# JohnsonLabJanelia/laserCalib

Hardware: NVIDIA B200
Metric: LM_iters_per_sec (higher is better)
Workload: dtype f64

## Files before the change

### include/lcba.h

```cpp
#ifndef LCBA_H
#define LCBA_H

#include <stddef.h>
#include <stdint.h>

#ifdef __cplusplus
extern "C" {
#endif

#define LCBA_VERSION 100
#define LCBA_CAM_PARAMS 11
#define LCBA_MAX_CAMERAS 64
#define LCBA_MAX_TRACE 512

enum {
  LCBA_OK = 0,
  LCBA_E_ARG = -1,
  LCBA_E_CUDA = -2,
  LCBA_E_STATE = -3,
  LCBA_E_UNSUPPORTED = -4,
  LCBA_E_NONFINITE = -5,
  LCBA_E_NCCL = -6
};

// ... 33 lines not shown

typedef struct lcba_result {
  double cost;
  double optimality;
  double initial_cost;
  int64_t nfev;
  int64_t njev;
  int64_t iterations;
  int32_t status;
  int32_t n_trace;
  double solve_ms;
  int64_t gpu_launches;
  double reserved[6];
} lcba_result;

typedef struct lcba_kernel_stat {
  char name[32];
  int64_t launches;
  double total_ms;
} lcba_kernel_stat;

int lcba_version(void);
int lcba_create(lcba_t** out, int device);
void lcba_destroy(lcba_t* h);
const char* lcba_last_error(const lcba_t* h);
void lcba_default_options(lcba_options* o);

int lcba_set_problem(lcba_t* h, int32_t C, int64_t P, int64_t N, const double* cams,
                     const double* pts, const double* obs_uv, const int64_t* cam_idx,
                     const int64_t* pt_idx, const double* weights_or_null);
int lcba_set_problem_shard(lcba_t* h, int32_t C, int64_t P, int64_t N, const double* cams,
                           const double* pts, const double* obs_uv, const int64_t* cam_idx,
                           const int64_t* pt_idx, const double* weights_or_null, int64_t pt_offset);
int lcba_set_params(lcba_t* h, const double* cams, const double* pts);
int lcba_get_params(lcba_t* h, double* cams_out, double* pts_out);

int lcba_rotate(lcba_t* h, int64_t M, const double* pts, const double* rot_vecs, double* out);
int lcba_project(lcba_t* h, int64_t M, const double* pts, const double* cams_rows,
                 double* out_uv);

int lcba_unproject(lcba_t* h, int64_t M, const double* uv, const double* Z, int64_t nZ,
                   const double* camera_matrix, const double* dist5, const double* rc_ext,
                   const double* tc_ext, double* out_xyz);

#define LCBA_SQ_CAMONLY 0
#define LCBA_SQ_TRANSFORM 1
int lcba_sq_normal(lcba_t* h, int32_t mode, const double* theta, double* cost_out, double* g_out,
                   double* H_out);

int lcba_residuals(lcba_t* h, const double* x_or_null, double* r_out, double* cost_out);

int lcba_jacobian_blocks(lcba_t* h, const double* x_or_null, double* Jc, double* Jp);

int lcba_sparsity_indices(lcba_t* h, int32_t C, int64_t P, int64_t N, const int64_t* cam_idx,
                          const int64_t* pt_idx, int32_t* indices_out);

int lcba_solve(lcba_t* h, const lcba_options* opt, lcba_result* res);
int lcba_get_trace(lcba_t* h, lcba_trace_row* rows, int32_t max_rows);
typedef void (*lcba_iteration_cb)(const lcba_trace_row* row, void* user);
int lcba_set_iteration_callback(lcba_t* h, lcba_iteration_cb cb, void* user);
int lcba_get_grad(lcba_t* h, double* g_out );
int lcba_get_profile(lcba_t* h, lcba_kernel_stat* stats, int32_t max_stats, int32_t* n_out);

int lcba_linearize(lcba_t* h, double lam, double* S_out, double* rhs_out, double* grad_out,
                   double* scale_inv_out, double* cost_out);

int lcba_time_device(lcba_t* h, int32_t what, int32_t reps, double* ms_out);

int lcba_nccl_unique_id(void* id_out128);
int lcba_comm_init(lcba_t* h, int32_t rank, int32_t nranks, const void* id128);

int lcba_debug_tr2d(double B00, double B01, double B11, double g0, double g1, double Delta,
                    double* p_out2, int* newton_out);

int lcba_debug_schur_stats(lcba_t* h, long long* out, int max_ctas, int* nkinds, int* nslices);

int lcba_debug_mma_plan(int32_t C, int32_t sm_count, int32_t* units_out, int32_t max_kinds,
                        int32_t* nslices_out, int32_t* ok_out);

int lcba_debug_i8_plan(int32_t C, int64_t P, int32_t sm_count, int32_t* tiles_out, int32_t max_tiles,
                       int32_t* work_out, int32_t max_work, int32_t* nwork_out, int32_t* nrg_out,
                       int64_t* nkb_out);

int lcba_debug_peer_reduce(lcba_t* h, int enable);

int lcba_host_is_nondecreasing_i64(const int64_t* v, int64_t n, int32_t threads);

#ifdef __cplusplus
}
#endif
#endif
```

### lasercalib_b200/_cabi.py

```python
from __future__ import annotations

import ctypes as C
import os

import numpy as np

_PKG = os.path.dirname(os.path.abspath(__file__))
LIB_PATH = os.path.join(_PKG, "liblcba.so")

LCBA_MAX_TRACE = 512
E_NAMES = {-1: "LCBA_E_ARG", -2: "LCBA_E_CUDA", -3: "LCBA_E_STATE", -4: "LCBA_E_UNSUPPORTED",
           -5: "LCBA_E_NONFINITE", -6: "LCBA_E_NCCL"}

SYMBOLS = ["lcba_version", "lcba_create", "lcba_destroy", "lcba_last_error", "lcba_default_options",
           "lcba_set_problem", "lcba_set_problem_shard", "lcba_set_params", "lcba_get_params", "lcba_rotate", "lcba_project",
           "lcba_unproject", "lcba_residuals", "lcba_jacobian_blocks", "lcba_sparsity_indices", "lcba_solve",
           "lcba_get_trace", "lcba_get_grad", "lcba_get_profile", "lcba_linearize",
           "lcba_time_device", "lcba_nccl_unique_id", "lcba_comm_init", "lcba_debug_tr2d",
           "lcba_sq_normal", "lcba_debug_schur_stats", "lcba_debug_mma_plan",
           "lcba_set_iteration_callback", "lcba_debug_i8_plan", "lcba_host_is_nondecreasing_i64", "lcba_debug_peer_reduce"]


class Options(C.Structure):
    _fields_ = [("ftol", C.c_double), ("xtol", C.c_double), ("gtol", C.c_double),
                ("max_nfev", C.c_int64), ("verbose", C.c_int32), ("profile", C.c_int32),
                ("max_iterations", C.c_int32), ("fix_cameras", C.c_int32), ("shared_intrinsics", C.c_int32), ("reserved", C.c_int32 * 3)]


class TraceRow(C.Structure):
    _fields_ = [("iteration", C.c_int64), ("nfev", C.c_int64), ("cost", C.c_double),
                ("cost_reduction", C.c_double), ("step_norm", C.c_double),
                ("optimality", C.c_double), ("delta", C.c_double), ("reg_term", C.c_double)]


class Result(C.Structure):
    _fields_ = [("cost", C.c_double), ("optimality", C.c_double), ("initial_cost", C.c_double),
                ("nfev", C.c_int64), ("njev", C.c_int64), ("iterations", C.c_int64),
                ("status", C.c_int32), ("n_trace", C.c_int32), ("solve_ms", C.c_double),
                ("gpu_launches", C.c_int64), ("reserved", C.c_double * 6)]


class KernelStat(C.Structure):
    _fields_ = [("name", C.c_char * 32), ("launches", C.c_int64), ("total_ms", C.c_double)]


ITERATION_CB = C.CFUNCTYPE(None, C.POINTER(TraceRow), C.c_void_p)


def _row_dict(r):
    return dict(iteration=r.iteration, nfev=r.nfev, cost=r.cost, cost_reduction=r.cost_reduction,
                step_norm=r.step_norm, optimality=r.optimality, delta=r.delta, reg_term=r.reg_term)


class LcbaError(RuntimeError):
    def __init__(self, code, msg):
        super().__init__("%s (%d): %s" % (E_NAMES.get(code, "LCBA_E_?"), code, msg))
        self.code = code


_lib = None


def load():
    global _lib
    if _lib is not None:
        return _lib
    if not os.path.exists(LIB_PATH):
        raise ImportError(
            "lasercalib_b200: %s is missing — build it with `python -m lasercalib_b200.build` "
            "(there is no CPU fallback)" % LIB_PATH)
    lib = C.CDLL(LIB_PATH, mode=C.RTLD_GLOBAL)
    vp, i32, i64, dbl = C.c_void_p, C.c_int32, C.c_int64, C.c_double
    pd = C.POINTER(C.c_double)
    lib.lcba_version.restype = C.c_int
    lib.lcba_create.argtypes = [C.POINTER(vp), C.c_int]
    lib.lcba_destroy.argtypes = [vp]
    lib.lcba_destroy.restype = None
    lib.lcba_last_error.argtypes = [vp]
    lib.lcba_last_error.restype = C.c_char_p
    lib.lcba_default_options.argtypes = [C.POINTER(Options)]
    lib.lcba_default_options.restype = None
    lib.lcba_set_problem.argtypes = [vp, i32, i64, i64, vp, vp, vp, vp, vp, vp]
    lib.lcba_set_problem_shard.argtypes = [vp, i32, i64, i64, vp, vp, vp, vp, vp, vp, i64]
    lib.lcba_set_params.argtypes = [vp, vp, vp]
    lib.lcba_get_params.argtypes = [vp, vp, vp]
    lib.lcba_rotate.argtypes = [vp, i64, vp, vp, vp]
    lib.lcba_project.argtypes = [vp, i64, vp, vp, vp]
    lib.lcba_unproject.argtypes = [vp, i64, vp, vp, i64, vp, vp, vp, vp, vp]
    lib.lcba_residuals.argtypes = [vp, vp, vp, pd]
    lib.lcba_jacobian_blocks.argtypes = [vp, vp, vp, vp]
    lib.lcba_sparsity_indices.argtypes = [vp, i32, i64, i64, vp, vp, vp]
    lib.lcba_solve.argtypes = [vp, C.POINTER(Options), C.POINTER(Result)]
    lib.lcba_get_trace.argtypes = [vp, C.POINTER(TraceRow), i32]
    lib.lcba_set_iteration_callback.argtypes = [vp, ITERATION_CB, vp]
    lib.lcba_get_grad.argtypes = [vp, vp]
    lib.lcba_get_profile.argtypes = [vp, C.POINTER(KernelStat), i32, C.POINTER(i32)]
    lib.lcba_linearize.argtypes = [vp, dbl, vp, vp, vp, vp, pd]
    lib.lcba_time_device.argtypes = [vp, i32, i32, pd]
    lib.lcba_nccl_unique_id.argtypes = [vp]
    lib.lcba_comm_init.argtypes = [vp, i32, i32, vp]
    lib.lcba_sq_normal.argtypes = [vp, i32, vp, pd, vp, vp]
    lib.lcba_debug_mma_plan.argtypes = [i32, i32, vp, i32, C.POINTER(i32), C.POINTER(i32)]
    lib.lcba_debug_schur_stats.argtypes = [vp, vp, C.c_int, C.POINTER(C.c_int), C.POINTER(C.c_int)]
    lib.lcba_debug_i8_plan.argtypes = [i32, i64, i32, vp, i32, vp, i32, C.POINTER(i32), C.POINTER(i32), C.POINTER(i64)]
    lib.lcba_host_is_nondecreasing_i64.argtypes = [vp, i64, i32]
    lib.lcba_debug_peer_reduce.argtypes = [vp, i32]
    lib.lcba_debug_tr2d.argtypes = [dbl, dbl, dbl, dbl, dbl, dbl, pd, C.POINTER(C.c_int)]
    _lib = lib
    return lib


def _ptr(a):
    return None if a is None else a.ctypes.data_as(C.c_void_p)


def _f64(a, shape=None):
    a = np.ascontiguousarray(a, dtype=np.float64)
    if shape is not None:
        a = a.reshape(shape)
    return a


def _i64(a):
    return np.ascontiguousarray(a, dtype=np.int64)


class Engine:

    def __init__(self, device=-1):
        self.lib = load()
        h = C.c_void_p()
        rc = self.lib.lcba_create(C.byref(h), int(device))
        if rc != 0:
            raise LcbaError(rc, self.lib.lcba_last_error(None).decode())
        self.h = h
        self.C = self.P = self.N = 0
        self.generation = 0

    def close(self):
        if getattr(self, "h", None):
            self.lib.lcba_destroy(self.h)
            self.h = None

    def __del__(self):
        try:
            self.close()
        except Exception:
            pass

    def _check(self, rc):
        if rc != 0:
            raise LcbaError(rc, self.lib.lcba_last_error(self.h).decode())

    def set_problem(self, cams, pts, points_2d, camera_ind, point_ind, weights=None, pt_offset=0):
        cams, pts = _f64(cams), _f64(pts)
        p2 = _f64(points_2d)
        ci, pi = _i64(camera_ind).ravel(), _i64(point_ind).ravel()
        w = None if weights is None else _f64(weights).ravel()
        if cams.ndim != 2 or cams.shape[1] != 11:
            raise ValueError("cameraArray must have shape (n_cameras, 11)")
        if pts.ndim != 2 or pts.shape[1] != 3:
            raise ValueError("points3D must have shape (n_points, 3)")
        N = ci.size
        if pi.size != N or p2.shape != (N, 2) or (w is not None and w.size != N):
            raise ValueError("observation arrays must share their first dimension")
        self._check(self.lib.lcba_set_problem_shard(self.h, cams.shape[0], pts.shape[0], N,
                                                    _ptr(cams), _ptr(pts), _ptr(p2), _ptr(ci),
                                                    _ptr(pi), _ptr(w), int(pt_offset)))
        self.C, self.P, self.N = cams.shape[0], pts.shape[0], N
        self.generation += 1

    def set_params(self, cams, pts):
        self.generation += 1
        cams, pts = _f64(cams, (self.C, 11)), _f64(pts, (self.P, 3))
        self._check(self.lib.lcba_set_params(self.h, _ptr(cams), _ptr(pts)))

    def get_params(self, x_out=None):
        if x_out is None:
            cams = np.empty((self.C, 11))
            pts = np.empty((self.P, 3))
        else:
            cams = x_out[: 11 * self.C].reshape(self.C, 11)
            pts = x_out[11 * self.C:].reshape(self.P, 3)
        self._check(self.lib.lcba_get_params(self.h, _ptr(cams), _ptr(pts)))
        return cams, pts

    def rotate(self, points, rot_vecs):
# ... 144 lines not shown
```

### lasercalib_b200/csrc/lcba.cu

```cuda
#include <dlfcn.h>
#include <math.h>
#include <stdio.h>
#include <string.h>
#include <algorithm>
#include <map>
#include <string>
#include <thread>
#include <vector>

#include <nvtx3/nvToolsExt.h>

#include "common.cuh"
#include "control.cuh"
#include "dense.cuh"
#include "eval.cuh"
#include "ingest.cuh"
#include "linearize.cuh"
#include "dense_passes.cuh"
#include "schur.cuh"
#include "schur_mma.cuh"
#include "schur_i8.cuh"
#include "peer_reduce.cuh"
#include "variants.cuh"

// ... 802 lines not shown
  NvtxRange nvtx_("lcba:linearize");
  const int C = h->C, w = h->cur;
  LCBA_TRY(build_tables(h, w));
  if (h->use_dense) {
    const size_t smem = dense_lin_smem_doubles(C) * 8;
    KL(h, "linearize", k_linearize_dense<<<h->dp_grid_lin, DP_THREADS, smem, h->stream>>>(
          h->d_tab[w], h->d_pts[w], h->d_uv, h->d_w, h->d_obs_start, h->d_mask, h->P, C, h->dp_pb,
          h->d_Vg, h->d_dpart, h->d_part));
    KL(h, "reduce", k_reduce_cols<<<nblk(C * DP_CAM_VALS, RC_COLS), RC_COLS * RC_ROWS, 0, h->stream>>>(
          h->d_dpart, h->dp_grid_lin, C * DP_CAM_VALS, h->d_dred));
    KL(h, "reduce", k_dense_cam_unpack<<<nblk(C * DP_CAM_VALS, 128), 128, 0, h->stream>>>(
          h->d_dred, C, h->d_camsum, h->d_U));
    KL(h, "reduce", k_reduce_scalars<<<1, 256, 0, h->stream>>>(h->d_part, h->dp_grid_lin, 1,
                                                               h->d_camsum + C * CAMSUM, 1));
  } else {
  const size_t smem = linearize_smem_doubles(C) * 8;
  KL(h, "linearize", k_linearize<<<h->lin_grid, LIN_THREADS, smem, h->stream>>>(
        h->d_tab[w], h->d_pts[w], h->d_uv, h->d_cam, h->d_pt, h->d_w, h->d_obs_start, h->d_bins,
        h->nbins, C, h->d_Vg, h->d_campart, h->d_part));
  KL(h, "reduce", k_reduce_cols<<<nblk(C * CAMSUM, RC_COLS), RC_COLS * RC_ROWS, 0, h->stream>>>(
        h->d_campart, h->lin_grid, C * CAMSUM, h->d_camsum));
  KL(h, "reduce", k_reduce_scalars<<<1, 256, 0, h->stream>>>(h->d_part, h->lin_grid, 1,
                                                             h->d_camsum + C * CAMSUM, 1));
  }
  double* pp = h->d_camsum + C * CAMSUM + 1;
  KL(h, "point_prep", k_point_prep<<<h->pt_grid, 256, 0, h->stream>>>(
        h->d_Vg, h->d_pts[w], h->d_scl_p, h->d_gt_p, h->P, first, h->d_part));
  KL(h, "reduce", k_reduce_scalars<<<PP_K, 256, 0, h->stream>>>(h->d_part, h->pt_grid, PP_K, pp, 3));
  LCBA_TRY(allreduce(h, h->d_camsum, (size_t)C * CAMSUM + 1 + 3, NCCL_SUM));
  LCBA_TRY(allreduce(h, pp + 3, 1, NCCL_MAX));
  KL(h, "ctl", k_ctl_lin<<<1, 256, 0, h->stream>>>(h->d_camsum, h->d_cams[w], h->d_scl_c, h->d_gt_c,
                                                   h->d_g_c, C, h->d_ctl, first, h->fix_cameras, h->shared_intr));
  KL(h, "ctl", k_ctl_lin2<<<1, 1, 0, h->stream>>>(pp, h->d_ctl, first));
  return check_launch(h, "linearize pass");
}

static int pass_jdot(lcba_t* h) {
  NvtxRange nvtx_("lcba:jdot");
  const int C = h->C, w = h->cur;
  const size_t smem = ((size_t)C * CAMTAB + (size_t)C * NCP) * 8;
  if (h->use_pt) {
    KL(h, "jdot", k_jdot_pt<<<h->ptp_grid, PT_THREADS, smem, h->stream>>>(
          h->d_tab[w], h->d_pts[w], h->d_w, h->d_obs_start, h->d_mask, h->d_gt_c, h->d_gt_p, h->P, C, h->d_part));
    KL(h, "reduce", k_reduce_scalars<<<1, 256, 0, h->stream>>>(h->d_part, h->ptp_grid, 1, h->d_red, 1));
  } else if (h->use_dense && h->pt_mode == 2) {
    KL(h, "jdot", k_jdot_dense<<<h->dp_grid, DP_THREADS, (size_t)C * CAMTAB * 8, h->stream>>>(
          h->d_tab[w], h->d_pts[w], h->d_w, h->d_obs_start, h->d_mask, h->d_gt_c, h->d_gt_p, h->P, C,
          h->dp_pb, h->d_part));
    KL(h, "reduce", k_reduce_scalars<<<1, 256, 0, h->stream>>>(h->d_part, h->dp_grid, 1, h->d_red, 1));
  } else {
  KL(h, "jdot", k_jdot<<<h->obs_grid, 256, smem, h->stream>>>(
        h->d_tab[w], h->d_pts[w], h->d_cam, h->d_pt, h->d_w, h->d_gt_c, h->d_gt_p, h->N, C, h->d_part));
  KL(h, "reduce", k_reduce_scalars<<<1, 256, 0, h->stream>>>(h->d_part, h->obs_grid, 1, h->d_red, 1));
  }
  LCBA_TRY(allreduce(h, h->d_red, 1, NCCL_SUM));
  KL(h, "ctl", k_ctl_reg<<<1, 1, 0, h->stream>>>(h->d_red, h->d_ctl));
  return check_launch(h, "jdot pass");
}

static int pass_schur(lcba_t* h, const double* lam_host_or_null) {
  NvtxRange nvtx_("lcba:schur");
  const int C = h->C, w = h->cur, n = C * NCP;
  const SchurPlan& pl = h->plan;
  const double lam_arg = lam_host_or_null ? *lam_host_or_null : 0.0;
  const Ctl* ctl_arg = lam_host_or_null ? nullptr : h->d_ctl;
  KL(h, "point_factor", k_point_factor<<<nblk(h->P, 256), 256, 0, h->stream>>>(
        h->d_Vg, h->d_scl_p, lam_arg, ctl_arg, h->P, h->d_Lz));
  if (h->use_mma) {
    const MmaPlan& mp = h->mplan;
    if (!h->use_dense) {
    const size_t smem_u = ((size_t)((C * CAMTAB + 1) & ~1) + (size_t)h->camn_pb * C) * 8;
    KL(h, "cam_normal", k_cam_normal<<<h->camn_grid, 256, smem_u, h->stream>>>(
          h->d_tab[w], h->d_pts[w], h->d_pair_w, h->d_pair_start, h->d_mask, h->P, C, h->camn_pb, h->d_Upart));
    KL(h, "reduce", k_reduce_cols<<<nblk(C * CAMN_VALS, RC_COLS), RC_COLS * RC_ROWS, 0, h->stream>>>(
          h->d_Upart, h->camn_grid, C * CAMN_VALS, h->d_U));
    }
    const int nt = (NCP * C + 1 + 7) / 8, last = nt - 6 * ((nt + 5) / 6 - 1);
    if (h->use_i8) {
      const I8Plan& ip = h->i8plan;
      const int RP = ip.NRG * 8;
      const size_t smem_rm = ((size_t)I8_GROUP_CAMS * CAMTAB + 192) * 4;
      KL(h, "i8_rowmax", k_i8_rowmax<<<dim3(h->i8_gx_max, h->i8_groups), 192, smem_rm, h->stream>>>(
            h->d_tab[w], h->d_pts[w], h->d_pair_w, h->d_pair_start, h->d_mask, h->d_Lz, h->P, C, RP, h->d_i8rmax));
      KL(h, "i8_rowmax", k_i8_rowexp<<<nblk(RP, 128), 128, 0, h->stream>>>(h->d_i8rmax, h->i8_gx_max, NCP * C + 1, RP, h->d_i8erow));
      KL(h, "make_Y", k_i8_make<<<dim3(h->i8_gx_make, h->i8_groups), 192, i8_make_smem_bytes(), h->stream>>>(
            h->d_tab[w], h->d_pts[w], h->d_pair_w, h->d_pair_start, h->d_mask, h->d_Lz, h->P, C, ip.NRG, h->d_i8erow,
            h->d_i8planes));
      if (h->i8_tma)
        KL(h, "schur", k_i8_syrk<true><<<(unsigned)ip.work.size(), I8_THREADS, ip.smem_bytes, h->stream>>>(
              h->i8maps, h->d_i8planes, ip.NRG, h->d_i8work, h->d_i8partial, h->d_fail, h->d_stats));
      else
        KL(h, "schur", k_i8_syrk<false><<<(unsigned)ip.work.size(), I8_THREADS, ip.smem_bytes, h->stream>>>(
              h->i8maps, h->d_i8planes, ip.NRG, h->d_i8work, h->d_i8partial, h->d_fail, h->d_stats));
      KL(h, "schur_reduce", k_i8_gather<<<dim3((unsigned)ip.tiles.size(), 16), 256, 0, h->stream>>>(
            h->d_i8partial, h->d_i8tiles, C, h->d_i8erow, pl.npairs, h->d_Sred));
      KL(h, "schur_reduce", k_add_cam_blocks<<<nblk(C * 121, 128), 128, 0, h->stream>>>(h->d_U, C, h->d_Sred));
    } else {
    if (h->d_Yg) {
      const int pbk = MAKEY_THREADS / C, rpk = mp.kinds[0].rp;
      const size_t smem_y = ((size_t)((C * CAMTAB + 1) & ~1) + (size_t)3 * pbk * rpk) * 8;
      const int grid_y = (int)std::min<long long>((h->P + pbk - 1) / pbk, (long long)h->sm_count * 5);
      KL(h, "make_Y", k_make_Y<<<grid_y, MAKEY_THREADS, smem_y, h->stream>>>(
            h->d_tab[w], h->d_pts[w], h->d_pair_w, h->d_pair_start, h->d_mask, h->d_Lz, h->P, C, mp.kinds[0].rp,
            h->d_Yg));
    }
#define LCBA_MMA_LAUNCH(L)                                                                          \
  do {                                                                                              \
    if (h->d_Yg)                                                                                    \
      KL(h, "schur", (k_schur_mma<L, true><<<dim3(mp.nslices, mp.nkinds), MMA_THREADS, mp.smem_bytes, h->stream>>>( \
            h->d_Yg, h->d_tab[w], h->d_pts[w], h->d_pair_w, h->d_pair_start, h->d_mask, h->d_Lz, h->P, h->n_pairs, C, \
            h->d_mkinds, mp.nslices, pl.part_stride, pl.npairs, h->d_Spart, h->d_stats)));          \
    else                                                                                            \
      KL(h, "schur", (k_schur_mma<L, false><<<dim3(mp.nslices, mp.nkinds), MMA_THREADS, mp.smem_bytes, h->stream>>>( \
            nullptr, h->d_tab[w], h->d_pts[w], h->d_pair_w, h->d_pair_start, h->d_mask, h->d_Lz, h->P, h->n_pairs, C, \
            h->d_mkinds, mp.nslices, pl.part_stride, pl.npairs, h->d_Spart, h->d_stats)));          \
  } while (0)
    switch (last) {
      case 1: LCBA_MMA_LAUNCH(1); break;
      case 2: LCBA_MMA_LAUNCH(2); break;
      case 3: LCBA_MMA_LAUNCH(3); break;
      case 4: LCBA_MMA_LAUNCH(4); break;
      case 5: LCBA_MMA_LAUNCH(5); break;
      default: LCBA_MMA_LAUNCH(6); break;
    }
#undef LCBA_MMA_LAUNCH
    KL(h, "schur_reduce", k_reduce_cols<<<nblk((long long)pl.part_stride, RC_COLS), RC_COLS * RC_ROWS, 0, h->stream>>>(
          h->d_Spart, mp.nslices, (int)pl.part_stride, h->d_Sred));
    KL(h, "schur_reduce", k_add_cam_blocks<<<nblk(C * 121, 128), 128, 0, h->stream>>>(h->d_U, C, h->d_Sred));
    }
  } else {
  dim3 grid(pl.nslices, pl.nkinds);
  const bool skip = (double)h->n_pairs < 0.8 * (double)h->P * C;
#define LCBA_SCHUR_LAUNCH(SK, NR)                                                                   \
  KL(h, "schur", (k_schur<SK, NR><<<grid, pl.max_threads, pl.smem_bytes, h->stream>>>(              \
        h->d_tab[w], h->d_pts[w], h->d_pair_w, h->d_pair_start, h->d_mask, h->d_Lz, h->P, h->n_pairs, C, \
        h->d_kinds, h->d_hws, pl.nslices, pl.part_stride, pl.npairs, h->d_Spart, h->d_stats)))
  if (pl.cfg != 1) { if (skip) LCBA_SCHUR_LAUNCH(true, 160); else LCBA_SCHUR_LAUNCH(false, 160); }
  else             { if (skip) LCBA_SCHUR_LAUNCH(true, 128); else LCBA_SCHUR_LAUNCH(false, 128); }
#undef LCBA_SCHUR_LAUNCH
  KL(h, "schur_reduce", k_reduce_cols<<<nblk((long long)pl.part_stride, RC_COLS), RC_COLS * RC_ROWS, 0, h->stream>>>(
        h->d_Spart, pl.nslices, (int)pl.part_stride, h->d_Sred));
  }
  LCBA_TRY(allreduce(h, h->d_Sred, pl.part_stride, NCCL_SUM));
  if (h->shared_intr) {
    const int nr = 3 + 8 * C;
    KL(h, "assemble", k_assemble_S_shared<<<nblk((long long)nr * nr, 256), 256, 0, h->stream>>>(
          h->d_Sred, C, pl.npairs, h->d_camsum, h->d_scl_c, h->d_ctl,
          lam_host_or_null ? *lam_host_or_null : 0.0, lam_host_or_null ? 0 : 1, h->d_S, h->d_rhs,
          h->d_scl_red));
  } else {
    KL(h, "assemble", k_assemble_S<<<nblk((long long)n * n, 256), 256, 0, h->stream>>>(
          h->d_Sred, C, pl.npairs, h->d_camsum, h->d_scl_c, lam_arg, ctl_arg, h->d_S, h->d_rhs));
  }
  return check_launch(h, "schur pass");
}

static int pass_camera_solve(lcba_t* h, double mu) {
  NvtxRange nvtx_("lcba:camera_solve");
  const int n = h->shared_intr ? 3 + 8 * h->C : h->C * NCP;
  LCBA_CUDA(h, cudaMemsetAsync(h->d_fail, 0, 2 * sizeof(int), h->stream));
  const double* scl = h->shared_intr ? h->d_scl_red : h->d_scl_c;
  double* out = h->shared_intr ? h->d_pred : h->d_pc;
  {
    KL(h, "chol_copy", k_copy_damped_rhs<<<nblk((long long)(n + 1) * n, 256), 256, 0, h->stream>>>(
          h->d_S, n, mu, scl, h->d_rhs, h->d_Lf));
    int tiles = 1;
    if (n > CH_NB) {
// ... 503 lines not shown
  if (!nccl_load(err)) { set_error(h, err); return LCBA_E_NCCL; }
  cudaSetDevice(h->device);
  if (!id128) {
    if (!g_comm || g_comm_rank != rank || g_comm_nranks != nranks || g_comm_device != h->device) {
      set_error(h, "lcba_comm_init: no matching process communicator to attach (pass a unique id first)");
      return LCBA_E_STATE;
    }
    h->comm = g_comm;
    h->rank = rank;
    h->nranks = nranks;
    return LCBA_OK;
  }
  ncclUniqueId id;
  memcpy(&id, id128, sizeof(id));
  ncclComm_t comm = nullptr;
  int rc = g_nccl.CommInitRank(&comm, nranks, id, rank);
  if (rc != 0) { set_error(h, std::string("ncclCommInitRank: ") + g_nccl.GetErrorString(rc)); return LCBA_E_NCCL; }
  if (g_comm) g_nccl.CommDestroy(g_comm);
  g_comm = comm;
  g_comm_rank = rank;
  g_comm_nranks = nranks;
  g_comm_device = h->device;
  h->comm = comm;
  h->rank = rank;
  h->nranks = nranks;
  peer_setup(h);
  return LCBA_OK;
}

extern "C" int lcba_debug_peer_reduce(lcba_t* h, int enable) {
  if (!h || !h->comm) return 0;
  cudaSetDevice(h->device);
  cudaStreamSynchronize(h->stream);
  g_peer.ok = g_peer_available && enable != 0;
  return g_peer.ok ? 1 : 0;
}

extern "C" int lcba_debug_schur_stats(lcba_t* h, long long* out, int max_ctas, int* nkinds, int* nslices) {
  if (!h || !h->d_stats || !out) return LCBA_E_STATE;
  const int nk = h->use_i8 ? 1 : (h->use_mma ? h->mplan.nkinds : h->plan.nkinds);
  const int ns = h->use_i8 ? (int)h->i8plan.work.size() : (h->use_mma ? h->mplan.nslices : h->plan.nslices);
  const int n = std::min(max_ctas, ns * nk);
  cudaMemcpy(out, h->d_stats, (size_t)n * 4 * sizeof(long long), cudaMemcpyDeviceToHost);
  *nkinds = nk;
  *nslices = ns;
  return LCBA_OK;
}

extern "C" int lcba_debug_mma_plan(int32_t C, int32_t sm_count, int32_t* units_out, int32_t max_kinds,
                                   int32_t* nslices_out, int32_t* ok_out) {
  if (C < 1 || C > LCBA_MAX_CAMERAS || !units_out) return LCBA_E_ARG;
  const MmaPlan pl = make_mma_plan(C, sm_count, 227 * 1024 - 2048);
  if (ok_out) *ok_out = (pl.nkinds > 0 && C <= MMA_MAX_CAMERAS) ? 1 : 0;
  if (nslices_out) *nslices_out = pl.nslices;
  for (int k = 0; k < pl.nkinds && k < max_kinds; ++k)
    for (int w = 0; w < MMA_CONS_WARPS; ++w) {
      const MmaUnit& u = pl.kinds[k].unit[w];
      int32_t* o = units_out + ((size_t)k * MMA_CONS_WARPS + w) * 5;
      o[0] = u.tr0; o[1] = u.tc0; o[2] = u.nr; o[3] = u.nc; o[4] = u.tri;
    }
  return pl.nkinds;
}

extern "C" int lcba_debug_i8_plan(int32_t C, int64_t P, int32_t sm_count, int32_t* tiles_out, int32_t max_tiles,
                                  int32_t* work_out, int32_t max_work, int32_t* nwork_out, int32_t* nrg_out,
                                  int64_t* nkb_out) {
  if (C < 1 || C > LCBA_MAX_CAMERAS || P < 1 || !tiles_out) return LCBA_E_ARG;
  const I8Plan pl = make_i8_plan(C, P, sm_count);
  for (size_t i = 0; i < pl.tiles.size() && (int)i < max_tiles; ++i) {
    const I8Tile& t = pl.tiles[i];
    int32_t* o = tiles_out + 8 * i;
    o[0] = t.m_rg0; o[1] = t.m_nrg; o[2] = t.n_rg0; o[3] = t.n_nrg; o[4] = t.n2_rg0; o[5] = t.n2_nrg; o[6] = t.w0; o[7] = t.nw;
  }
  if (work_out)
    for (size_t i = 0; i < pl.work.size() && (int)i < max_work; ++i) {
      work_out[3 * i] = (int32_t)i; work_out[3 * i + 1] = pl.work[i].kb0; work_out[3 * i + 2] = pl.work[i].kb1;
    }
  if (nwork_out) *nwork_out = (int32_t)pl.work.size();
  if (nrg_out) *nrg_out = pl.NRG;
  if (nkb_out) *nkb_out = pl.nkb;
  return (int)pl.tiles.size();
}

extern "C" int lcba_sq_normal(lcba_t* h, int32_t mode, const double* theta, double* cost_out,
                              double* g_out, double* H_out) {
  if (!h || !h->have_problem) { set_error(h, "lcba_sq_normal: no problem set"); return LCBA_E_STATE; }
  if (!theta || (mode != LCBA_SQ_CAMONLY && mode != LCBA_SQ_TRANSFORM) || ((g_out == nullptr) != (H_out == nullptr))) {
    set_error(h, "lcba_sq_normal: bad mode, NULL theta, or only one of g / H given");
    return LCBA_E_ARG;
  }
  cudaSetDevice(h->device);
  const int C = h->C;
  const bool derivs = g_out != nullptr;
  const int K = (mode == LCBA_SQ_CAMONLY ? C * SQC_VALS : SQT_VALS) + 1;
  const int warps = sq_camonly_warps(C, h->smem_optin);
  const int threads = (mode == LCBA_SQ_CAMONLY) ? warps * 32 : SQ_THREADS;
  const int per_sm = (mode == LCBA_SQ_CAMONLY) ? 1 : 2;
  const int grid = (int)std::max<long long>(1, std::min<long long>((h->N + threads - 1) / threads,
                                                                   (long long)h->sm_count * per_sm));
  if (!h->d_sqpart || h->sq_grid < grid || h->sq_K < K) {
    LCBA_TRY(dev_alloc(h, &h->d_sqpart, (size_t)grid * K));
    LCBA_TRY(dev_alloc(h, &h->d_sqout, (size_t)K));
    if (!h->d_theta) LCBA_TRY(dev_alloc(h, &h->d_theta, 16));
    h->sq_grid = grid;
    h->sq_K = K;
  }
  const int cur = h->cur, scratch = 1 - h->cur;
  if (mode == LCBA_SQ_CAMONLY) {
    LCBA_CUDA(h, cudaMemcpyAsync(h->d_cams[scratch], theta, (size_t)C * NCP * 8, cudaMemcpyHostToDevice, h->stream));
    LCBA_TRY(build_tables(h, scratch));
    const size_t smem = ((size_t)((C * CAMTAB + 1) & ~1) + (derivs ? (size_t)warps * C * SQC_VALS : 0)) * 8;
    if (derivs)
      KL(h, "sq_camonly", k_sq_camonly<true><<<grid, threads, smem, h->stream>>>(
            h->d_tab[scratch], h->d_pts[cur], h->d_uv, h->d_cam, h->d_pt, h->d_w, h->N, C, h->d_sqpart));
    else
      KL(h, "sq_camonly_cost", k_sq_camonly<false><<<grid, threads, smem, h->stream>>>(
            h->d_tab[scratch], h->d_pts[cur], h->d_uv, h->d_cam, h->d_pt, h->d_w, h->N, C, h->d_sqpart));
  } else {
    LCBA_CUDA(h, cudaMemcpyAsync(h->d_theta, theta, 12 * 8, cudaMemcpyHostToDevice, h->stream));
    LCBA_TRY(build_tables(h, cur));
    const size_t smem = (size_t)((C * CAMTAB + 1) & ~1) * 8;
    if (derivs)
      KL(h, "sq_transform", k_sq_transform<true><<<grid, threads, smem, h->stream>>>(
            h->d_tab[cur], h->d_pts[cur], h->d_uv, h->d_cam, h->d_pt, h->d_w, h->N, C, h->d_theta, h->d_sqpart));
    else
      KL(h, "sq_transform_cost", k_sq_transform<false><<<grid, threads, smem, h->stream>>>(
            h->d_tab[cur], h->d_pts[cur], h->d_uv, h->d_cam, h->d_pt, h->d_w, h->N, C, h->d_theta, h->d_sqpart));
  }
  KL(h, "reduce", k_reduce_cols<<<nblk(K, RC_COLS), RC_COLS * RC_ROWS, 0, h->stream>>>(h->d_sqpart, grid, K, h->d_sqout));
  std::vector<double> v((size_t)K);
  LCBA_CUDA(h, cudaMemcpyAsync(v.data(), h->d_sqout, (size_t)K * 8, cudaMemcpyDeviceToHost, h->stream));
  LCBA_CUDA(h, cudaStreamSynchronize(h->stream));
  LCBA_TRY(check_launch(h, "lcba_sq_normal"));
  if (cost_out) *cost_out = 0.5 * v[K - 1];
  if (!derivs) return LCBA_OK;
  if (mode == LCBA_SQ_CAMONLY) {
    for (int c = 0; c < C; ++c) {
      const double* s = v.data() + (size_t)c * SQC_VALS;
      double* Hc = H_out + (size_t)c * NCP * NCP;
      int idx = 0;
      for (int a = 0; a < NCP; ++a)
        for (int b = a; b < NCP; ++b, ++idx) Hc[a * NCP + b] = Hc[b * NCP + a] = s[idx];
      for (int a = 0; a < NCP; ++a) g_out[(size_t)c * NCP + a] = s[66 + a];
    }
  } else {
    int mi[3][3], qi[4][4], n = 0;
    for (int k = 0; k < 3; ++k) for (int l = k; l < 3; ++l) mi[k][l] = mi[l][k] = n++;
    n = 0;
    for (int j = 0; j < 4; ++j) for (int i = j; i < 4; ++i) qi[j][i] = qi[i][j] = n++;
    for (int k = 0; k < 3; ++k)
      for (int j = 0; j < 4; ++j)
        for (int l = 0; l < 3; ++l)
          for (int i = 0; i < 4; ++i)
            H_out[(4 * k + j) * 12 + 4 * l + i] = v[(size_t)mi[k][l] * SQT_Q + qi[j][i]];
    for (int a = 0; a < 12; ++a) g_out[a] = v[60 + a];
  }
  return LCBA_OK;
}

extern "C" int lcba_debug_tr2d(double B00, double B01, double B11, double g0, double g1, double Delta,
                               double* p_out, int* newton_out) {
  if (!p_out) return LCBA_E_ARG;
  const TR2 t = solve_tr2d(B00, B01, B11, g0, g1, Delta);
  p_out[0] = t.p0;
  p_out[1] = t.p1;
  if (newton_out) *newton_out = t.newton;
// ... 27 lines not shown
```

### lasercalib_b200/csrc/schur_i8.cuh

```cuda
#pragma once
#include <cuda.h>
#include <algorithm>
#include <vector>
#include "common.cuh"
#include "schur_mma.cuh"

namespace lcba {

constexpr int I8_NS = 6;
constexpr int I8_DMAX = 6;
constexpr int I8_ND = I8_DMAX + 1;
constexpr int I8_PTS = 21;
constexpr int I8_STAGES = 3;
constexpr int I8_FLUSH = 224;
constexpr int I8_THREADS = 192;
constexpr int I8_RG_BYTES = 512;
constexpr int I8_GROUP_CAMS = 8;
constexpr int I8_GROUP_RG = 13;
constexpr int I8_GROUP_ROWS = I8_GROUP_RG * 8;

struct I8Work {
  int m_rg0, m_nrg, n_rg0, n_nrg, n2_rg0, n2_nrg;
  int kb0, kb1;
  int map_a, map_b1, map_b2, pad;
// ... 100 lines not shown
    if (r != CUDA_SUCCESS) return false;
  }
  return true;
}

__device__ __forceinline__ void i8_tma_4d(uint32_t dst, const CUtensorMap* map, int c0, int c1, int c2, int c3, uint32_t bar) {
  asm volatile("cp.async.bulk.tensor.4d.shared::cluster.global.mbarrier::complete_tx::bytes [%0], [%1, {%2, %3, %4, %5}], [%6];"
               ::"r"(dst), "l"(map), "r"(c0), "r"(c1), "r"(c2), "r"(c3), "r"(bar) : "memory");
}
__device__ __forceinline__ uint32_t i8_smem_u32(const void* p) { return (uint32_t)__cvta_generic_to_shared(p); }
__device__ __forceinline__ void i8_mbar_init(uint32_t bar, uint32_t count) {
  asm volatile("mbarrier.init.shared::cta.b64 [%0], %1;" ::"r"(bar), "r"(count) : "memory");
}
__device__ __forceinline__ void i8_mbar_expect_tx(uint32_t bar, uint32_t bytes) {
  asm volatile("mbarrier.arrive.expect_tx.shared::cta.b64 _, [%0], %1;" ::"r"(bar), "r"(bytes) : "memory");
}
__device__ __forceinline__ void i8_mbar_arrive(uint32_t bar) {
  asm volatile("mbarrier.arrive.shared::cta.b64 _, [%0];" ::"r"(bar) : "memory");
}
template <bool BACKOFF>
__device__ __forceinline__ void i8_mbar_wait(uint32_t bar, uint32_t parity, int* fail) {
  const long long t0 = clock64();
  while (true) {
    uint32_t ok;
    asm volatile("{\n\t.reg .pred p;\n\tmbarrier.try_wait.parity.shared::cta.b64 p, [%1], %2;\n\tselp.u32 %0, 1, 0, p;\n\t}"
                 : "=r"(ok) : "r"(bar), "r"(parity) : "memory");
    if (ok) return;
    if (BACKOFF) __nanosleep(128);
    if (clock64() - t0 > 6000000000LL) { atomicOr(fail, 4); asm volatile("trap;"); }
  }
}
__device__ __forceinline__ void i8_bulk_g2s(uint32_t dst, const void* src, uint32_t bytes, uint32_t bar) {
  asm volatile("cp.async.bulk.shared::cluster.global.mbarrier::complete_tx::bytes [%0], [%1], %2, [%3];"
               ::"r"(dst), "l"(src), "r"(bytes), "r"(bar) : "memory");
}
template <int COLL>
__device__ __forceinline__ void i8_mma(uint32_t tmem_d, uint64_t adesc, uint64_t bdesc, uint32_t idesc, uint32_t acc) {
#define I8_MMA_ASM(Q)                                                                                      \
  asm volatile("{\n\t.reg .pred p;\n\tsetp.ne.b32 p, %4, 0;\n\t"                                          \
               "tcgen05.mma.cta_group::1.kind::i8" Q " [%0], %1, %2, %3, {%5, %5, %5, %5}, p;\n\t}"         \
               ::"r"(tmem_d), "l"(adesc), "l"(bdesc), "r"(idesc), "r"(acc), "r"(0u) : "memory")
  if (COLL == 1) I8_MMA_ASM(".collector::a::fill");
  else if (COLL == 2) I8_MMA_ASM(".collector::a::use");
  else if (COLL == 3) I8_MMA_ASM(".collector::a::lastuse");
  else I8_MMA_ASM("");
#undef I8_MMA_ASM
}
__device__ __forceinline__ void i8_commit(uint32_t bar) {
  asm volatile("tcgen05.commit.cta_group::1.mbarrier::arrive::one.shared::cluster.b64 [%0];" ::"r"(bar) : "memory");
}
__device__ __forceinline__ bool i8_elect_one() {
  uint32_t p;
  asm volatile("{\n\t.reg .pred q;\n\telect.sync _|q, 0xffffffff;\n\tselp.u32 %0, 1, 0, q;\n\t}" : "=r"(p));
  return p != 0;
}
__device__ __forceinline__ void i8_tmem_ld16(uint32_t taddr, uint32_t (&v)[16]) {
  asm volatile("tcgen05.ld.sync.aligned.32x32b.x16.b32 "
               "{%0, %1, %2, %3, %4, %5, %6, %7, %8, %9, %10, %11, %12, %13, %14, %15}, [%16];"
               : "=r"(v[0]), "=r"(v[1]), "=r"(v[2]), "=r"(v[3]), "=r"(v[4]), "=r"(v[5]), "=r"(v[6]), "=r"(v[7]),
                 "=r"(v[8]), "=r"(v[9]), "=r"(v[10]), "=r"(v[11]), "=r"(v[12]), "=r"(v[13]), "=r"(v[14]), "=r"(v[15])
               : "r"(taddr) : "memory");
}

__device__ __forceinline__ void i8_item_values(const double* __restrict__ T, const double (&X)[3],
                                               const double (&li)[9], double w, bool live, double (&y)[3][NCP]) {
  ObsLin L;
  obs_linearize<false>(T, X[0], X[1], X[2], 0.0, 0.0, w, L, live);
  double Q[2][3];
#pragma unroll
  for (int i = 0; i < 2; ++i) {
    Q[i][0] = L.Jp[i][0] * li[0];
    Q[i][1] = fma(L.Jp[i][0], li[1], L.Jp[i][1] * li[2]);
    Q[i][2] = fma(L.Jp[i][0], li[3], fma(L.Jp[i][1], li[4], L.Jp[i][2] * li[5]));
  }
#pragma unroll
  for (int k = 0; k < 3; ++k) {
#pragma unroll
    for (int a = 0; a < 9; ++a) y[k][a] = fma(L.Jc[0][a], Q[0][k], L.Jc[1][a] * Q[1][k]);
    y[k][9] = w * Q[0][k];
    y[k][10] = w * Q[1][k];
  }
}

__device__ __forceinline__ void i8_item_absmax_f32(const float* __restrict__ T, float X, float Y, float Z,
                                                   const float (&li)[6], float w, float (&m)[NCP]) {
  const float* R = T + CT_R;
  const float xc = fmaf(R[0], X, fmaf(R[1], Y, fmaf(R[2], Z, T[3])));
  const float yc = fmaf(R[3], X, fmaf(R[4], Y, fmaf(R[5], Z, T[4])));
  const float zc = fmaf(R[6], X, fmaf(R[7], Y, fmaf(R[8], Z, T[5])));
  const float iz = 1.0f / zc;
  const float x = xc * iz, y = yc * iz;
  const float n = x * x + y * y;
  const float f = T[6], k1 = T[7], k2 = T[8];
  const float d = 1.0f + n * (k1 + k2 * n);
  const float dp = k1 + 2.0f * k2 * n;
  const float wf = w * f;
  const float e00 = wf * (d + 2.0f * x * x * dp), e01 = wf * (2.0f * x * y * dp), e11 = wf * (d + 2.0f * y * y * dp);
  float G[2][3] = {{e00 * iz, e01 * iz, -(e00 * x + e01 * y) * iz}, {e01 * iz, e11 * iz, -(e01 * x + e11 * y) * iz}};
  float Jc[2][9], Jp[2][3];
#pragma unroll
  for (int i = 0; i < 2; ++i)
#pragma unroll
    for (int j = 0; j < 3; ++j) Jp[i][j] = fmaf(G[i][0], R[j], fmaf(G[i][1], R[3 + j], G[i][2] * R[6 + j]));
  const float* Jr = T + CT_JR;
#pragma unroll
  for (int k = 0; k < 3; ++k) {
    const float c0 = Jr[k], c1 = Jr[3 + k], c2 = Jr[6 + k];
    const float m0 = fmaf(Y, c2, -Z * c1), m1 = fmaf(Z, c0, -X * c2), m2 = fmaf(X, c1, -Y * c0);
    Jc[0][k] = -fmaf(Jp[0][0], m0, fmaf(Jp[0][1], m1, Jp[0][2] * m2));
    Jc[1][k] = -fmaf(Jp[1][0], m0, fmaf(Jp[1][1], m1, Jp[1][2] * m2));
  }
#pragma unroll
  for (int i = 0; i < 2; ++i) { Jc[i][3] = G[i][0]; Jc[i][4] = G[i][1]; Jc[i][5] = G[i][2]; }
  const float wd = w * d, wfn = wf * n, wfn2 = wfn * n;
  Jc[0][6] = wd * x;   Jc[1][6] = wd * y;
  Jc[0][7] = wfn * x;  Jc[1][7] = wfn * y;
  Jc[0][8] = wfn2 * x; Jc[1][8] = wfn2 * y;
  float Q[2][3];
#pragma unroll
  for (int i = 0; i < 2; ++i) {
    Q[i][0] = Jp[i][0] * li[0];
    Q[i][1] = fmaf(Jp[i][0], li[1], Jp[i][1] * li[2]);
    Q[i][2] = fmaf(Jp[i][0], li[3], fmaf(Jp[i][1], li[4], Jp[i][2] * li[5]));
  }
#pragma unroll
  for (int k = 0; k < 3; ++k) {
#pragma unroll
    for (int a = 0; a < 9; ++a) m[a] = fmaxf(m[a], fabsf(fmaf(Jc[0][a], Q[0][k], Jc[1][a] * Q[1][k])));
    m[9] = fmaxf(m[9], fabsf(w * Q[0][k]));
    m[10] = fmaxf(m[10], fabsf(w * Q[1][k]));
  }
}

__global__ void __launch_bounds__(192, 4)
k_i8_rowmax(const double* __restrict__ tab, const double* __restrict__ pts, const double* __restrict__ wgt,
            const uint32_t* __restrict__ obs_start, const unsigned long long* __restrict__ mask,
            const double* __restrict__ Lz, long long P, int C, int RP, double* __restrict__ rmax_part) {
  extern __shared__ double s_dyn[];
  float* s_tab = reinterpret_cast<float*>(s_dyn);
  float* s_red = s_tab + I8_GROUP_CAMS * CAMTAB;
  const int t = threadIdx.x, g = blockIdx.y;
  const int c0 = g * I8_GROUP_CAMS, gc = min(I8_GROUP_CAMS, C - c0);
  for (int i = t; i < gc * CAMTAB; i += blockDim.x) s_tab[i] = (float)tab[c0 * CAMTAB + i];
  __syncthreads();
  const bool worker = t < I8_PTS * gc;
  const int q = worker ? t / gc : 0, cl = worker ? t % gc : 0, cam = c0 + cl;
  const bool zthread = (g == gridDim.y - 1) && t >= 168 && t < 168 + I8_PTS;
  float mx[NCP], mz = 0.0f;
#pragma unroll
  for (int a = 0; a < NCP; ++a) mx[a] = 0.0f;
  const long long nkb = (P + I8_PTS - 1) / I8_PTS;
  for (long long kb = blockIdx.x; kb < nkb; kb += gridDim.x) {
    if (worker) {
      const long long p = kb * I8_PTS + q;
      if (p < P) {
        const unsigned long long m = mask[p];
        if ((m >> cam) & 1ull) {
          const float w = wgt ? (float)wgt[(long long)obs_start[p] + __popcll(m & ((1ull << cam) - 1ull))] : 1.0f;
          float li[6];
#pragma unroll
          for (int a = 0; a < 6; ++a) li[a] = (float)Lz[p * 9 + a];
          i8_item_absmax_f32(s_tab + cl * CAMTAB, (float)pts[3 * p], (float)pts[3 * p + 1], (float)pts[3 * p + 2], li, w, mx);
        }
      }
    }
    if (zthread) {
      const long long p = kb * I8_PTS + (t - 168);
      if (p < P) mz = fmaxf(mz, fmaxf(fabsf((float)Lz[p * 9 + 6]), fmaxf(fabsf((float)Lz[p * 9 + 7]), fabsf((float)Lz[p * 9 + 8]))));
    }
  }
  double* out = rmax_part + (size_t)blockIdx.x * RP;
#pragma unroll
  for (int a = 0; a < NCP; ++a) {
    __syncthreads();
    s_red[t] = worker ? mx[a] : 0.0f;
    __syncthreads();
    if (t < gc) {
      float m = 0.0f;
      for (int qq = 0; qq < I8_PTS; ++qq) m = fmaxf(m, s_red[qq * gc + t]);
      out[(c0 + t) * NCP + a] = (double)m;
    }
  }
  if (g == gridDim.y - 1) {
    __syncthreads();
    s_red[t] = zthread ? mz : 0.0f;
    __syncthreads();
    if (t == 0) {
      float m = 0.0f;
      for (int i = 168; i < 168 + I8_PTS; ++i) m = fmaxf(m, s_red[i]);
      out[NCP * C] = (double)m;
    }
  }
}

__global__ void k_i8_rowexp(const double* __restrict__ rmax_part, int nb, int R, int RP, int* __restrict__ e_row) {
  const int r = blockIdx.x * blockDim.x + threadIdx.x;
  if (r >= RP) return;
  double m = 0.0;
  if (r < R) for (int b = 0; b < nb; ++b) m = fmax(m, rmax_part[(size_t)b * RP + r]);
  int e = 0;
  if (m > 0.0 && m < 1e300) { frexp(m * 1.001, &e); e += 2; }
  e_row[r] = e;
}

__device__ __forceinline__ unsigned long long i8_encode(double v, double scale) {
  const long long T = __double2ll_rn(v * scale);
  return (unsigned long long)(T + 0x808080808080LL) ^ 0x808080808080ULL;
}

constexpr int I8_VAL_LD = 65;
inline size_t i8_make_smem_bytes() {
  return (size_t)I8_GROUP_CAMS * CAMTAB * 8 + (size_t)I8_GROUP_ROWS * 8 + (size_t)I8_GROUP_ROWS * I8_VAL_LD * 8;
}

__global__ void __launch_bounds__(192, 3)
k_i8_make(const double* __restrict__ tab, const double* __restrict__ pts, const double* __restrict__ wgt,
          const uint32_t* __restrict__ obs_start, const unsigned long long* __restrict__ mask,
          const double* __restrict__ Lz, long long P, int C, int NRG, const int* __restrict__ e_row,
          unsigned char* __restrict__ planes) {
  extern __shared__ __align__(16) unsigned char s_raw[];
  double* s_tab = reinterpret_cast<double*>(s_raw);
  double* s_scale = s_tab + I8_GROUP_CAMS * CAMTAB;
  unsigned long long* s_val = reinterpret_cast<unsigned long long*>(s_scale + I8_GROUP_ROWS);
  const int t = threadIdx.x, g = blockIdx.y, lane = t & 31, wid = t >> 5;
  const int c0 = g * I8_GROUP_CAMS, gc = min(I8_GROUP_CAMS, C - c0);
  const int rg0 = 11 * g;
  const int nrgl = (g == (int)gridDim.y - 1) ? NRG - rg0 : 11;
  for (int i = t; i < gc * CAMTAB; i += blockDim.x) s_tab[i] = tab[c0 * CAMTAB + i];
  for (int i = t; i < I8_GROUP_ROWS; i += blockDim.x)
    s_scale[i] = (rg0 * 8 + i < NRG * 8) ? ldexp(1.0, 8 * I8_NS - e_row[rg0 * 8 + i]) : 0.0;
  for (int i = t; i < I8_GROUP_ROWS * I8_VAL_LD; i += blockDim.x) s_val[i] = 0ull;
  __syncthreads();
  const bool worker = t < I8_PTS * gc;
  const int slot = worker ? t / gc : 0;
  const int q = slot < 16 ? (slot >> 1) + 8 * (slot & 1) : slot, cl = worker ? t % gc : 0, cam = c0 + cl;
  const bool zthread = (g == (int)gridDim.y - 1) && t >= 168 && t < 168 + I8_PTS;
  const int zrow = NCP * C - rg0 * 8;
  const long long nkb = (P + I8_PTS - 1) / I8_PTS;
  unsigned long long n_m = 0ull;
  double n_X[3] = {0, 0, 0}, n_li[6] = {0, 0, 0, 0, 0, 0};
  auto prefetch = [&](long long kb) {
    n_m = 0ull;
    const long long p = kb * I8_PTS + q;
    if (worker && kb < nkb && p < P) {
      n_m = mask[p];
#pragma unroll
      for (int a = 0; a < 3; ++a) n_X[a] = pts[3 * p + a];
#pragma unroll
      for (int a = 0; a < 6; ++a) n_li[a] = Lz[p * 9 + a];
    }
  };
  prefetch(blockIdx.x);
  for (long long kb = blockIdx.x; kb < nkb; kb += gridDim.x) {
    if (worker) {
      const long long p = kb * I8_PTS + q;
      const unsigned long long m = n_m;
      const bool live = (m >> cam) & 1ull;
      double X[3], li[6];
#pragma unroll
      for (int a = 0; a < 3; ++a) X[a] = n_X[a];
#pragma unroll
      for (int a = 0; a < 6; ++a) li[a] = n_li[a];
      prefetch(kb + gridDim.x);
      unsigned long long* dst = s_val + (size_t)(cl * NCP) * I8_VAL_LD + 3 * q;
      if (live) {
        const double w = wgt ? wgt[(long long)obs_start[p] + __popcll(m & ((1ull << cam) - 1ull))] : 1.0;
        ObsLin L;
        obs_linearize<false>(s_tab + cl * CAMTAB, X[0], X[1], X[2], 0.0, 0.0, w, L);
        const double* sc = s_scale + cl * NCP;
#pragma unroll
        for (int k = 0; k < 3; ++k) {
          double q0, q1;
          if (k == 0) { q0 = L.Jp[0][0] * li[0]; q1 = L.Jp[1][0] * li[0]; }
          else if (k == 1) { q0 = fma(L.Jp[0][0], li[1], L.Jp[0][1] * li[2]); q1 = fma(L.Jp[1][0], li[1], L.Jp[1][1] * li[2]); }
          else { q0 = fma(L.Jp[0][0], li[3], fma(L.Jp[0][1], li[4], L.Jp[0][2] * li[5]));
                 q1 = fma(L.Jp[1][0], li[3], fma(L.Jp[1][1], li[4], L.Jp[1][2] * li[5])); }
#pragma unroll
          for (int a = 0; a < 9; ++a) dst[a * I8_VAL_LD + k] = i8_encode(fma(L.Jc[0][a], q0, L.Jc[1][a] * q1), sc[a]);
          dst[9 * I8_VAL_LD + k] = i8_encode(w * q0, sc[9]);
          dst[10 * I8_VAL_LD + k] = i8_encode(w * q1, sc[10]);
        }
      } else {
#pragma unroll
        for (int k = 0; k < 3; ++k)
#pragma unroll
          for (int a = 0; a < NCP; ++a) dst[a * I8_VAL_LD + k] = 0ull;
      }
    }
    if (zthread) {
      const int qq = t - 168;
// ... 285 lines not shown
```

Baseline: 126.2.

## Vectorize i8 absmax with paired float ops, warp-per-row exponent reduce, faster encode

```diff
diff --git a/include/lcba.h b/include/lcba.h
--- a/include/lcba.h
+++ b/include/lcba.h
@@ -139,6 +139,8 @@
                        int32_t* work_out, int32_t max_work, int32_t* nwork_out, int32_t* nrg_out,
                        int64_t* nkb_out);
 
+int lcba_debug_i8_operands(lcba_t* h, uint8_t* planes_out, int32_t* e_row_out);
+
 int lcba_debug_peer_reduce(lcba_t* h, int enable);
 
 int lcba_host_is_nondecreasing_i64(const int64_t* v, int64_t n, int32_t threads);
diff --git a/lasercalib_b200/_cabi.py b/lasercalib_b200/_cabi.py
--- a/lasercalib_b200/_cabi.py
+++ b/lasercalib_b200/_cabi.py
@@ -18,7 +18,7 @@
            "lcba_get_trace", "lcba_get_grad", "lcba_get_profile", "lcba_linearize",
            "lcba_time_device", "lcba_nccl_unique_id", "lcba_comm_init", "lcba_debug_tr2d",
            "lcba_sq_normal", "lcba_debug_schur_stats", "lcba_debug_mma_plan",
-           "lcba_set_iteration_callback", "lcba_debug_i8_plan", "lcba_host_is_nondecreasing_i64", "lcba_debug_peer_reduce"]
+           "lcba_set_iteration_callback", "lcba_debug_i8_plan", "lcba_debug_i8_operands", "lcba_host_is_nondecreasing_i64", "lcba_debug_peer_reduce"]
 
 
 class Options(C.Structure):
@@ -103,6 +103,7 @@
     lib.lcba_debug_mma_plan.argtypes = [i32, i32, vp, i32, C.POINTER(i32), C.POINTER(i32)]
     lib.lcba_debug_schur_stats.argtypes = [vp, vp, C.c_int, C.POINTER(C.c_int), C.POINTER(C.c_int)]
     lib.lcba_debug_i8_plan.argtypes = [i32, i64, i32, vp, i32, vp, i32, C.POINTER(i32), C.POINTER(i32), C.POINTER(i64)]
+    lib.lcba_debug_i8_operands.argtypes = [vp, vp, vp]
     lib.lcba_host_is_nondecreasing_i64.argtypes = [vp, i64, i32]
     lib.lcba_debug_peer_reduce.argtypes = [vp, i32]
     lib.lcba_debug_tr2d.argtypes = [dbl, dbl, dbl, dbl, dbl, dbl, pd, C.POINTER(C.c_int)]
diff --git a/lasercalib_b200/csrc/lcba.cu b/lasercalib_b200/csrc/lcba.cu
--- a/lasercalib_b200/csrc/lcba.cu
+++ b/lasercalib_b200/csrc/lcba.cu
@@ -908,7 +908,7 @@
       const size_t smem_rm = ((size_t)I8_GROUP_CAMS * CAMTAB + 192) * 4;
       KL(h, "i8_rowmax", k_i8_rowmax<<<dim3(h->i8_gx_max, h->i8_groups), 192, smem_rm, h->stream>>>(
             h->d_tab[w], h->d_pts[w], h->d_pair_w, h->d_pair_start, h->d_mask, h->d_Lz, h->P, C, RP, h->d_i8rmax));
-      KL(h, "i8_rowmax", k_i8_rowexp<<<nblk(RP, 128), 128, 0, h->stream>>>(h->d_i8rmax, h->i8_gx_max, NCP * C + 1, RP, h->d_i8erow));
+      KL(h, "i8_rowmax", k_i8_rowexp<<<nblk(RP, I8_ROWEXP_THREADS / 32), I8_ROWEXP_THREADS, 0, h->stream>>>(h->d_i8rmax, h->i8_gx_max, NCP * C + 1, RP, h->d_i8erow));
       KL(h, "make_Y", k_i8_make<<<dim3(h->i8_gx_make, h->i8_groups), 192, i8_make_smem_bytes(), h->stream>>>(
             h->d_tab[w], h->d_pts[w], h->d_pair_w, h->d_pair_start, h->d_mask, h->d_Lz, h->P, C, ip.NRG, h->d_i8erow,
             h->d_i8planes));
@@ -1578,6 +1578,16 @@
   return (int)pl.tiles.size();
 }
 
+extern "C" int lcba_debug_i8_operands(lcba_t* h, uint8_t* planes_out, int32_t* e_row_out) {
+  if (!h || !h->use_i8 || !h->d_i8planes) return LCBA_E_STATE;
+  if (!planes_out || !e_row_out) return LCBA_E_ARG;
+  cudaSetDevice(h->device);
+  LCBA_CUDA(h, cudaMemcpyAsync(planes_out, h->d_i8planes, h->i8plan.plane_bytes, cudaMemcpyDeviceToHost, h->stream));
+  LCBA_CUDA(h, cudaMemcpyAsync(e_row_out, h->d_i8erow, (size_t)h->i8plan.NRG * 8 * sizeof(int32_t), cudaMemcpyDeviceToHost, h->stream));
+  LCBA_CUDA(h, cudaStreamSynchronize(h->stream));
+  return LCBA_OK;
+}
+
 extern "C" int lcba_sq_normal(lcba_t* h, int32_t mode, const double* theta, double* cost_out,
                               double* g_out, double* H_out) {
   if (!h || !h->have_problem) { set_error(h, "lcba_sq_normal: no problem set"); return LCBA_E_STATE; }
diff --git a/lasercalib_b200/csrc/schur_i8.cuh b/lasercalib_b200/csrc/schur_i8.cuh
--- a/lasercalib_b200/csrc/schur_i8.cuh
+++ b/lasercalib_b200/csrc/schur_i8.cuh
@@ -206,6 +206,7 @@
   }
 }
 
+__device__ __forceinline__ float2 i8_f2(float s) { return make_float2(s, s); }
 __device__ __forceinline__ void i8_item_absmax_f32(const float* __restrict__ T, float X, float Y, float Z,
                                                    const float (&li)[6], float w, float (&m)[NCP]) {
   const float* R = T + CT_R;
@@ -220,40 +221,39 @@
   const float dp = k1 + 2.0f * k2 * n;
   const float wf = w * f;
   const float e00 = wf * (d + 2.0f * x * x * dp), e01 = wf * (2.0f * x * y * dp), e11 = wf * (d + 2.0f * y * y * dp);
-  float G[2][3] = {{e00 * iz, e01 * iz, -(e00 * x + e01 * y) * iz}, {e01 * iz, e11 * iz, -(e01 * x + e11 * y) * iz}};
-  float Jc[2][9], Jp[2][3];
-#pragma unroll
-  for (int i = 0; i < 2; ++i)
-#pragma unroll
-    for (int j = 0; j < 3; ++j) Jp[i][j] = fmaf(G[i][0], R[j], fmaf(G[i][1], R[3 + j], G[i][2] * R[6 + j]));
+  const float2 G[3] = {__fmul2_rn(make_float2(e00, e01), i8_f2(iz)), __fmul2_rn(make_float2(e01, e11), i8_f2(iz)),
+                       make_float2(-(e00 * x + e01 * y) * iz, -(e01 * x + e11 * y) * iz)};
+  float2 Jc[9], Jp[3];
+#pragma unroll
+  for (int j = 0; j < 3; ++j)
+    Jp[j] = __ffma2_rn(G[0], i8_f2(R[j]), __ffma2_rn(G[1], i8_f2(R[3 + j]), __fmul2_rn(G[2], i8_f2(R[6 + j]))));
   const float* Jr = T + CT_JR;
 #pragma unroll
   for (int k = 0; k < 3; ++k) {
     const float c0 = Jr[k], c1 = Jr[3 + k], c2 = Jr[6 + k];
     const float m0 = fmaf(Y, c2, -Z * c1), m1 = fmaf(Z, c0, -X * c2), m2 = fmaf(X, c1, -Y * c0);
-    Jc[0][k] = -fmaf(Jp[0][0], m0, fmaf(Jp[0][1], m1, Jp[0][2] * m2));
-    Jc[1][k] = -fmaf(Jp[1][0], m0, fmaf(Jp[1][1], m1, Jp[1][2] * m2));
-  }
-#pragma unroll
-  for (int i = 0; i < 2; ++i) { Jc[i][3] = G[i][0]; Jc[i][4] = G[i][1]; Jc[i][5] = G[i][2]; }
+    Jc[k] = __ffma2_rn(Jp[0], i8_f2(m0), __ffma2_rn(Jp[1], i8_f2(m1), __fmul2_rn(Jp[2], i8_f2(m2))));
+  }
+  Jc[3] = G[0]; Jc[4] = G[1]; Jc[5] = G[2];
   const float wd = w * d, wfn = wf * n, wfn2 = wfn * n;
-  Jc[0][6] = wd * x;   Jc[1][6] = wd * y;
-  Jc[0][7] = wfn * x;  Jc[1][7] = wfn * y;
-  Jc[0][8] = wfn2 * x; Jc[1][8] = wfn2 * y;
-  float Q[2][3];
-#pragma unroll
-  for (int i = 0; i < 2; ++i) {
-    Q[i][0] = Jp[i][0] * li[0];
-    Q[i][1] = fmaf(Jp[i][0], li[1], Jp[i][1] * li[2]);
-    Q[i][2] = fmaf(Jp[i][0], li[3], fmaf(Jp[i][1], li[4], Jp[i][2] * li[5]));
-  }
-#pragma unroll
-  for (int k = 0; k < 3; ++k) {
-#pragma unroll
-    for (int a = 0; a < 9; ++a) m[a] = fmaxf(m[a], fabsf(fmaf(Jc[0][a], Q[0][k], Jc[1][a] * Q[1][k])));
-    m[9] = fmaxf(m[9], fabsf(w * Q[0][k]));
-    m[10] = fmaxf(m[10], fabsf(w * Q[1][k]));
-  }
+  const float2 xy = make_float2(x, y);
+  Jc[6] = __fmul2_rn(i8_f2(wd), xy);
+  Jc[7] = __fmul2_rn(i8_f2(wfn), xy);
+  Jc[8] = __fmul2_rn(i8_f2(wfn2), xy);
+  float2 Q[3];
+  Q[0] = __fmul2_rn(Jp[0], i8_f2(li[0]));
+  Q[1] = __ffma2_rn(Jp[0], i8_f2(li[1]), __fmul2_rn(Jp[1], i8_f2(li[2])));
+  Q[2] = __ffma2_rn(Jp[0], i8_f2(li[3]), __ffma2_rn(Jp[1], i8_f2(li[4]), __fmul2_rn(Jp[2], i8_f2(li[5]))));
+  const float2 Q01r0 = make_float2(Q[0].x, Q[1].x), Q01r1 = make_float2(Q[0].y, Q[1].y);
+#pragma unroll
+  for (int a = 0; a < 9; ++a) {
+    const float2 v = __ffma2_rn(i8_f2(Jc[a].x), Q01r0, __fmul2_rn(i8_f2(Jc[a].y), Q01r1));
+    const float v2 = fmaf(Jc[a].x, Q[2].x, Jc[a].y * Q[2].y);
+    m[a] = fmaxf(m[a], fmaxf(fmaxf(fabsf(v.x), fabsf(v.y)), fabsf(v2)));
+  }
+  const float2 w0 = __fmul2_rn(i8_f2(w), Q01r0), w1 = __fmul2_rn(i8_f2(w), Q01r1);
+  m[9] = fmaxf(m[9], fmaxf(fmaxf(fabsf(w0.x), fabsf(w0.y)), fabsf(w * Q[2].x)));
+  m[10] = fmaxf(m[10], fmaxf(fmaxf(fabsf(w1.x), fabsf(w1.y)), fabsf(w * Q[2].y)));
 }
 
 __global__ void __launch_bounds__(192, 4)
@@ -317,19 +317,23 @@
   }
 }
 
-__global__ void k_i8_rowexp(const double* __restrict__ rmax_part, int nb, int R, int RP, int* __restrict__ e_row) {
-  const int r = blockIdx.x * blockDim.x + threadIdx.x;
+constexpr int I8_ROWEXP_THREADS = 128;
+__global__ void __launch_bounds__(I8_ROWEXP_THREADS)
+k_i8_rowexp(const double* __restrict__ rmax_part, int nb, int R, int RP, int* __restrict__ e_row) {
+  const int r = blockIdx.x * (I8_ROWEXP_THREADS / 32) + (threadIdx.x >> 5), lane = threadIdx.x & 31;
   if (r >= RP) return;
   double m = 0.0;
-  if (r < R) for (int b = 0; b < nb; ++b) m = fmax(m, rmax_part[(size_t)b * RP + r]);
+  if (r < R) for (int b = lane; b < nb; b += 32) m = fmax(m, rmax_part[(size_t)b * RP + r]);
+#pragma unroll
+  for (int o = 16; o > 0; o >>= 1) m = fmax(m, __shfl_xor_sync(0xffffffffu, m, o));
   int e = 0;
   if (m > 0.0 && m < 1e300) { frexp(m * 1.001, &e); e += 2; }
-  e_row[r] = e;
+  if (lane == 0) e_row[r] = e;
 }
 
 __device__ __forceinline__ unsigned long long i8_encode(double v, double scale) {
-  const long long T = __double2ll_rn(v * scale);
-  return (unsigned long long)(T + 0x808080808080LL) ^ 0x808080808080ULL;
+  const double x = __dadd_rn(__dmul_rn(v, scale), 6755399441055744.0);
+  return ((unsigned long long)__double_as_longlong(x) + (0x808080808080ULL - 0x4338000000000000ULL)) ^ 0x808080808080ULL;
 }
 
 constexpr int I8_VAL_LD = 65;
```

Result: no change. 127.5, median of 6 (+1.0%).
